# seanome/kmerseek

Hardware: NVIDIA B200
Metric: residues/s sketched+indexed (higher is better)
Workload: dtype u64

## Files before the change

### kmerseek_b200/csrc/dense.cu

```cuda
#include <cub/device/device_radix_sort.cuh>
#include <cub/device/device_scan.cuh>

#include <algorithm>
#include <cmath>

#include "common.cuh"
#include "dense.cuh"
#include "dense_scatter.cuh"
#include "index_build.cuh"
#include "sketch.cuh"

namespace ks {

namespace {

__device__ uint64_t murmur_of_pattern(uint32_t pattern, uint32_t k) {
    uint64_t w[3] = {0, 0, 0};
    for (uint32_t j = 0; j < k; j++) w[j >> 3] |= (uint64_t)(((pattern >> j) & 1u) ? 'h' : 'p') << (8 * (j & 7));
    uint64_t h1 = SEED, h2 = SEED;
    const uint32_t nb = k / 16, rem = k % 16;
    if (nb) {
        h1 ^= mix_k1(w[0]);
        h1 = rotl64(h1, 27) + h2;
        h1 = h1 * 5 + 0x52dce729;
        h2 ^= mix_k2(w[1]);
        h2 = rotl64(h2, 31) + h1;
        h2 = h2 * 5 + 0x38495ab5;
    }
    const uint64_t t1 = w[2 * nb], t2 = nb ? 0 : w[1];
    if (rem > 8) h2 ^= mix_k2(t2);
    if (rem > 0) h1 ^= mix_k1(t1);
    h1 ^= k;
    h2 ^= k;
    h1 += h2;
    h2 += h1;
    h1 = fmix64(h1);
    h2 = fmix64(h2);
    return h1 + h2;
}

__device__ __forceinline__ uint32_t hp_translate(uint32_t c) {
    constexpr uint32_t H = (1u << 0) | (1u << 5) | (1u << 6) | (1u << 8) | (1u << 11) | (1u << 12) | (1u << 15) | (1u << 21) |
                           (1u << 22) | (1u << 24);
    constexpr uint32_t P = (1u << 2) | (1u << 3) | (1u << 4) | (1u << 7) | (1u << 10) | (1u << 13) | (1u << 16) | (1u << 17) |
                           (1u << 18) | (1u << 19);
    if (c == '*') return '*';
    const uint32_t i = c - 'A';
    if (i < 26u) {
        if ((H >> i) & 1u) return 'h';
        if ((P >> i) & 1u) return 'p';
    }
    return 'X';
}

__device__ __noinline__ uint64_t dense_window_hash(const uint8_t* __restrict__ res, int packed, uint64_t g, uint32_t k) {
    uint64_t w[3] = {0, 0, 0};
    for (uint32_t j = 0; j < k; j++) {
        const uint64_t i = g + j;
        uint32_t c;
        if (packed) {
            const uint64_t byte = (i >> 3) * 5;
            uint64_t v = 0;
            for (int t = 0; t < 5; t++) v |= (uint64_t)res[byte + t] << (8 * t);
            const uint32_t code = (uint32_t)(v >> (5 * (i & 7))) & 31u;
            c = code == 0 ? 0u : code <= 26 ? 'A' + code - 1 : code == 27 ? (uint32_t)'*' : 0u;
        } else {
            c = res[i];
        }
        w[j >> 3] |= (uint64_t)hp_translate(c) << (8 * (j & 7));
    }
    uint64_t h1 = SEED, h2 = SEED;
    const uint32_t nb = k / 16, rem = k % 16;
    if (nb) {
        h1 ^= mix_k1(w[0]);
        h1 = rotl64(h1, 27) + h2;
        h1 = h1 * 5 + 0x52dce729;
        h2 ^= mix_k2(w[1]);
        h2 = rotl64(h2, 31) + h1;
        h2 = h2 * 5 + 0x38495ab5;
    }
    const uint64_t t1 = w[2 * nb], t2 = nb ? 0 : w[1];
    if (rem > 8) h2 ^= mix_k2(t2);
    if (rem > 0) h1 ^= mix_k1(t1);
    h1 ^= k;
    h2 ^= k;
    h1 += h2;
    h2 += h1;
    h1 = fmix64(h1);
    h2 = fmix64(h2);
    return h1 + h2;
}

__global__ void dense_hash_codes_kernel(uint32_t k, uint64_t* __restrict__ hash, uint32_t* __restrict__ code) {
    const uint32_t c = blockIdx.x * blockDim.x + threadIdx.x;
    if (c >= (1u << k)) return;
    hash[c] = murmur_of_pattern(c, k);
    code[c] = c;
}

__global__ void dense_group_base_kernel(uint32_t n, const uint64_t* __restrict__ sorted_hash, uint32_t* __restrict__ group_base) {
    const uint32_t p = blockIdx.x * blockDim.x + threadIdx.x;
    if (p > (1u << DENSE_PREFIX_BITS)) return;
    if (p == (1u << DENSE_PREFIX_BITS)) { group_base[p] = n; return; }
    const uint64_t lim = (uint64_t)p << (64 - DENSE_PREFIX_BITS);
    uint32_t lo = 0, hi = n;
    while (lo < hi) {
        const uint32_t mid = (lo + hi) >> 1;
        if (sorted_hash[mid] < lim) lo = mid + 1; else hi = mid;
    }
    group_base[p] = lo;
}

__global__ void dense_check_kernel(uint32_t n, const uint64_t* __restrict__ sorted_hash, const uint32_t* __restrict__ group_base,
                                   uint32_t* __restrict__ flags) {
    const uint32_t r = blockIdx.x * blockDim.x + threadIdx.x;
    if (r >= n) return;
    const uint64_t h = sorted_hash[r];
    if (h == 0 || (r && sorted_hash[r - 1] == h)) atomicOr(flags, 1u);
    atomicMax(flags + 3, r - group_base[(uint32_t)(h >> (64 - DENSE_PREFIX_BITS))]);
}

__global__ void dense_code_kernel(uint32_t n, const uint64_t* __restrict__ sorted_hash, const uint32_t* __restrict__ pattern_of_rank,
                                  const uint32_t* __restrict__ group_base, int rb, int parity, uint32_t* __restrict__ code_of_pattern) {
    const uint32_t r = blockIdx.x * blockDim.x + threadIdx.x;
    if (r >= n) return;
    const uint32_t pfx = (uint32_t)(sorted_hash[r] >> (64 - DENSE_PREFIX_BITS));
    const uint32_t local = r - group_base[pfx];
    code_of_pattern[pattern_of_rank[r]] = (pfx << rb) | (parity ? 2u * local + 1u : local);
}

__global__ void dense_windows_kernel(const uint64_t* __restrict__ offsets, uint32_t n_prot, uint32_t k,
                                     uint32_t* __restrict__ t_abund, uint32_t* __restrict__ t_size) {
    const uint32_t p = blockIdx.x * blockDim.x + threadIdx.x;
    if (p >= n_prot) return;
    const uint64_t len = offsets[p + 1] - offsets[p];
    const uint32_t w = len >= k ? (uint32_t)(len - k + 1) : 0u;
    t_abund[p] = w;
    t_size[p] = w;
}

__device__ __forceinline__ uint64_t hash_of_code(uint32_t code, int rb, int parity, const uint32_t* __restrict__ group_base,
                                                 const uint64_t* __restrict__ sorted_hash) {
    return sorted_hash[group_base[code >> rb] + ((code & ((1u << rb) - 1u)) >> parity)];
}

constexpr int DC_THREADS = 256;
constexpr int DC_ROWS = 8;
constexpr int DC_TILE = DC_THREADS * DC_ROWS;

__global__ void __launch_bounds__(DC_THREADS)
dense_count_kernel(const uint64_t* __restrict__ keys, uint64_t n, int loc_bits, int pos_bits, uint64_t* __restrict__ tile_counts) {
    __shared__ uint32_t s_k[DC_THREADS / 32], s_g[DC_THREADS / 32];
    const uint32_t tid = threadIdx.x, lane = tid & 31, warp = tid >> 5;
    const uint64_t base = (uint64_t)blockIdx.x * DC_TILE;
    uint32_t ck = 0, cg = 0;
#pragma unroll
    for (int r = 0; r < DC_ROWS; r++) {
        const uint64_t i = base + (uint64_t)(warp * DC_ROWS + r) * 32 + lane;
        bool hk = false, hg = false;
        const uint64_t key = i < n ? keys[i] : 0ull;
        uint64_t prev = __shfl_up_sync(0xffffffffu, key, 1);
        if (i < n) {
            if (lane == 0) prev = i ? keys[i - 1] : ~key;
            hk = (key >> loc_bits) != (prev >> loc_bits);
            hg = (key >> pos_bits) != (prev >> pos_bits);
        }
        ck += __popc(__ballot_sync(0xffffffffu, hk));
        cg += __popc(__ballot_sync(0xffffffffu, hg));
    }
    if (lane == 0) { s_k[warp] = ck; s_g[warp] = cg; }
    __syncthreads();
    if (tid == 0) {
        uint32_t k = 0, g = 0;
        for (int w = 0; w < DC_THREADS / 32; w++) { k += s_k[w]; g += s_g[w]; }
        tile_counts[blockIdx.x] = (uint64_t)k | ((uint64_t)g << 32);
        if (blockIdx.x == gridDim.x - 1) tile_counts[gridDim.x] = 0;
    }
}

__global__ void __launch_bounds__(DC_THREADS)
dense_write_kernel(const uint64_t* __restrict__ keys_in, uint64_t n, int loc_bits, int pos_bits, const uint64_t* __restrict__ tile_prefix,
                   const uint64_t* __restrict__ sorted_hash, const uint32_t* __restrict__ group_base, int rb, int parity,
                   uint64_t* __restrict__ loc, uint64_t* __restrict__ keys,
                   uint32_t* __restrict__ key_grp, uint32_t* __restrict__ grp_start, uint32_t* __restrict__ t_size,
                   uint64_t* __restrict__ d_counts) {
    __shared__ uint32_t s_k[DC_THREADS / 32], s_g[DC_THREADS / 32];
    const uint32_t tid = threadIdx.x, lane = tid & 31, warp = tid >> 5;
    const uint32_t lt = (1u << lane) - 1u;
    const uint64_t base = (uint64_t)blockIdx.x * DC_TILE;
    const uint64_t pos_mask = (1ull << pos_bits) - 1ull, pid_mask = (1ull << (loc_bits - pos_bits)) - 1ull;
    uint64_t key[DC_ROWS];
    uint32_t bk[DC_ROWS], bg[DC_ROWS];
    uint32_t wk = 0, wg = 0;
#pragma unroll
    for (int r = 0; r < DC_ROWS; r++) {
        const uint64_t i = base + (uint64_t)(warp * DC_ROWS + r) * 32 + lane;
        bool hk = false, hg = false;
        key[r] = i < n ? keys_in[i] : 0ull;
        uint64_t prev = __shfl_up_sync(0xffffffffu, key[r], 1);
        if (i < n) {
            if (lane == 0) prev = i ? keys_in[i - 1] : ~key[r];
            hk = (key[r] >> loc_bits) != (prev >> loc_bits);
            hg = (key[r] >> pos_bits) != (prev >> pos_bits);
            const uint32_t pid = (uint32_t)((key[r] >> pos_bits) & pid_mask);
            loc[i] = ((uint64_t)pid << 32) | (key[r] & pos_mask);
            if (!hg) atomicSub(&t_size[pid], 1u);
        }
        bk[r] = __ballot_sync(0xffffffffu, hk);
        bg[r] = __ballot_sync(0xffffffffu, hg);
        wk += __popc(bk[r]);
        wg += __popc(bg[r]);
    }
    if (lane == 0) { s_k[warp] = wk; s_g[warp] = wg; }
    __syncthreads();
    const uint64_t pfx = tile_prefix[blockIdx.x];
    uint32_t rk = (uint32_t)pfx, rg = (uint32_t)(pfx >> 32);
    uint32_t tk = 0, tg = 0;
#pragma unroll
    for (int w = 0; w < DC_THREADS / 32; w++) {
        if (w < (int)warp) { rk += s_k[w]; rg += s_g[w]; }
        tk += s_k[w];
        tg += s_g[w];
    }
#pragma unroll
    for (int r = 0; r < DC_ROWS; r++) {
        const uint64_t i = base + (uint64_t)(warp * DC_ROWS + r) * 32 + lane;
        const uint32_t g = rg + __popc(bg[r] & lt);
        if ((bg[r] >> lane) & 1u) grp_start[g] = (uint32_t)i;
        if ((bk[r] >> lane) & 1u) {
            const uint32_t u = rk + __popc(bk[r] & lt);
            keys[u] = hash_of_code((uint32_t)(key[r] >> loc_bits), rb, parity, group_base, sorted_hash);
            key_grp[u] = g;
        }
        rk += __popc(bk[r]);
        rg += __popc(bg[r]);
    }
    if (blockIdx.x == gridDim.x - 1 && tid == 0) {
        const uint64_t U = (uint32_t)pfx + tk, G = (uint32_t)(pfx >> 32) + tg;
        d_counts[0] = U;
        d_counts[1] = G;
        key_grp[U] = (uint32_t)G;
        grp_start[G] = (uint32_t)n;
    }
}

#ifndef KS_DP_CTAS
#define KS_DP_CTAS 5
#endif
__global__ void __launch_bounds__(DS_THREADS, KS_DP_CTAS)
dense_partition_kernel(const uint64_t* __restrict__ region1, uint32_t cap1, const uint2* __restrict__ chunk_map, DenseScatter sc) {
    __shared__ DenseScatterSmem s_sc;
    __shared__ uint64_t s_dst[DS_TILE];
    const uint2 e = chunk_map[blockIdx.x];
    const uint32_t nv = e.x >> 16, b1 = e.x & 0xffffu;
    if (nv == 0) return;
    const uint64_t* src = region1 + (uint64_t)b1 * cap1 + e.y;
    uint64_t key[DS_ITEMS];
    uint32_t valid = 0;
#pragma unroll
    for (int it = 0; it < DS_ITEMS; it++) {
        const uint32_t i = it * DS_THREADS + threadIdx.x;
        key[it] = 0;
        if (i < nv) { key[it] = src[i]; valid |= 1u << it; }
    }
    scatter_keys(key, valid, sc, b1 << sc.bits, s_sc, s_dst);
}

#ifndef KS_DB_THREADS
#define KS_DB_THREADS 512
#endif
constexpr int DB_THREADS = KS_DB_THREADS;
constexpr int DB_CTAS = 2048 / DB_THREADS;
constexpr int DB_WARPS = DB_THREADS / 32;
constexpr int DB_CAP = 4096;
constexpr int DB_ROWS = DB_CAP / DB_THREADS;
constexpr int DB_BIN_BITS = 13;
constexpr int DB_BINS = 1 << DB_BIN_BITS;
constexpr int DB_WORDS_PER_THREAD = DB_BINS / 2 / DB_THREADS;
#ifdef KS_DB_NOSLICE
constexpr int DB_HASH_SLICE = 0;
#else
constexpr int DB_HASH_SLICE = 512;
#endif
constexpr size_t DB_SMEM = (size_t)DB_CAP * 8 + (size_t)DB_BINS * 2 + (size_t)DB_HASH_SLICE * 8;
constexpr uint32_t DB_BIN_SORT_MAX = 32;
constexpr int DB_SLOT_BITS = 12;
static_assert(DB_WORDS_PER_THREAD % 4 == 0 && DB_ROWS * DB_WARPS == 128, "scan layout");

struct DenseBucketArgs {
    const uint64_t* region2;
    const uint32_t* cursor2;
    const uint32_t* bstart;
    uint32_t nb;
    int bucket_bits;
    int rem_bits;
    int loc_bits, pos_bits;
    int rb, parity;
    const uint64_t* sorted_hash;
    const uint32_t* group_base;
    uint64_t* loc;
    uint64_t* keys;
    uint32_t *key_grp, *grp_start, *t_size;
    uint64_t* counts;
    unsigned long long* d_counts;
    uint32_t* dir;
    int dir_sub, dir_shift;
    const uint8_t* residues;
    const uint64_t* offsets;
    int packed;
    uint32_t k;
    const uint32_t* exc_flag;
    const uint32_t* skip_flag;
};

template <bool EXC>
__global__ void __launch_bounds__(DB_THREADS, DB_CTAS)
dense_bucket_kernel(DenseBucketArgs a) {
    extern __shared__ __align__(16) unsigned char smem_raw[];
    uint64_t* B = reinterpret_cast<uint64_t*>(smem_raw);
    uint32_t* cnt = reinterpret_cast<uint32_t*>(B + DB_CAP);
    uint64_t* s_hash = reinterpret_cast<uint64_t*>(cnt + DB_BINS / 2);
    uint64_t* s_keyh = reinterpret_cast<uint64_t*>(cnt);
    constexpr uint32_t KEYH_CAP = DB_BINS / 4;
    const uint16_t* off16 = reinterpret_cast<const uint16_t*>(cnt);
    __shared__ uint32_t s_wsum[DB_WARPS];
    __shared__ uint32_t s_cw[DB_ROWS * DB_WARPS];
    __shared__ uint32_t s_tk, s_tg;
    const uint32_t tid = threadIdx.x, lane = tid & 31, warp = tid >> 5;
    const uint32_t lt = (1u << lane) - 1u;
    if (*a.skip_flag != 0) return;
    if ((*a.exc_flag != 0) != EXC) return;
    const int up = 64 - a.rem_bits;
    const int rrb = a.rem_bits - a.loc_bits;
    const int pb = up + a.loc_bits;
    const bool squeeze = a.parity && pb >= 64 - DB_BIN_BITS && pb < 63;
    const int n_low = squeeze ? DB_BIN_BITS - (63 - pb) : 0;
    auto bin_of = [&](uint64_t it) -> uint32_t {
        if (!squeeze) return (uint32_t)(it >> (64 - DB_BIN_BITS));
        return (uint32_t)(((it >> (pb + 1)) << n_low) | ((it >> (pb - n_low)) & ((1ull << n_low) - 1ull)));
    };
    const int rank_sh = up + a.loc_bits, grp_sh = up + a.pos_bits;
    const uint64_t pos_mask = (1ull << a.pos_bits) - 1ull, pid_mask = (1ull << (a.loc_bits - a.pos_bits)) - 1ull;
    constexpr uint64_t SLOT_MASK = (1ull << DB_SLOT_BITS) - 1ull;
    const uint32_t dir_n = 1u << a.dir_sub;
    auto dir_local = [&](uint64_t h) -> int32_t { return (int32_t)((uint32_t)(h >> a.dir_shift) & (dir_n - 1u)); };
    for (uint32_t b = blockIdx.x; b < a.nb; b += gridDim.x) {
    __syncthreads();
    for (uint32_t i = tid; i < DB_BINS / 8; i += DB_THREADS) reinterpret_cast<uint4*>(cnt)[i] = make_uint4(0, 0, 0, 0);
    const uint64_t* src = a.region2 + (uint64_t)b * DB_CAP;
    uint64_t item[DB_ROWS];
    constexpr int SPEC_ROWS = DB_ROWS / 2;
#pragma unroll
    for (int r = 0; r < SPEC_ROWS; r++) item[r] = src[r * DB_THREADS + tid];
    const uint32_t m = min(a.cursor2[b], (uint32_t)DB_CAP);
    const uint32_t s0 = a.bstart[b];
    const uint32_t kb = s0 + b;
    uint32_t* dir_b = a.dir + (uint64_t)b * (dir_n + 1u);
    const uint32_t pshift = DENSE_PREFIX_BITS - a.bucket_bits;
    const uint32_t slice_base = a.group_base[b << pshift];
    const uint32_t slice_n = a.group_base[(b + 1) << pshift] - slice_base;
    const bool hash_slice = DB_HASH_SLICE > 0 && slice_n <= (uint32_t)DB_HASH_SLICE;
    if (hash_slice) for (uint32_t i = tid; i < slice_n; i += DB_THREADS) s_hash[i] = a.sorted_hash[slice_base + i];
    if (m == 0) {
        if (tid == 0) { a.key_grp[kb] = kb; a.grp_start[kb] = s0; a.counts[b] = 0; }
        for (uint32_t x = tid; x <= dir_n; x += DB_THREADS) dir_b[x] = kb;
        continue;
    }
#pragma unroll
    for (int r = SPEC_ROWS; r < DB_ROWS; r++) {
        if (r * DB_THREADS >= m) break;
        const uint32_t j = r * DB_THREADS + tid;
        if (j < m) item[r] = src[j];
    }
    __syncthreads();
#pragma unroll
    for (int r = 0; r < DB_ROWS; r++) {
        const uint32_t j = r * DB_THREADS + tid;
        if (r * DB_THREADS >= m) break;
        if (j < m) {
            item[r] <<= up;
            const uint32_t bin = bin_of(item[r]), sh16 = 16 * (bin & 1u);
            item[r] |= (atomicAdd(&cnt[bin >> 1], 1u << sh16) >> sh16) & 0xffffu;
        }
    }
    __syncthreads();
    bool big_bin = false;
    {
        uint32_t w[DB_WORDS_PER_THREAD];
#pragma unroll
        for (int q = 0; q < DB_WORDS_PER_THREAD / 4; q++) {
            const uint4 c = reinterpret_cast<uint4*>(cnt)[tid * (DB_WORDS_PER_THREAD / 4) + q];
            w[4 * q] = c.x; w[4 * q + 1] = c.y; w[4 * q + 2] = c.z; w[4 * q + 3] = c.w;
        }
        uint32_t total = 0;
#pragma unroll
        for (int i = 0; i < DB_WORDS_PER_THREAD; i++) {
            const uint32_t lo = w[i] & 0xffffu, hi = w[i] >> 16;
            total += lo + hi;
            big_bin |= lo > DB_BIN_SORT_MAX || hi > DB_BIN_SORT_MAX;
        }
        uint32_t incl = total;
#pragma unroll
        for (int o = 1; o < 32; o <<= 1) {
            const uint32_t v = __shfl_up_sync(0xffffffffu, incl, o);
            if ((int)lane >= o) incl += v;
        }
        if (lane == 31) s_wsum[warp] = incl;
        __syncthreads();
        uint32_t off = 0;
#pragma unroll
        for (int w2 = 0; w2 < DB_WARPS; w2++) off += w2 < (int)warp ? s_wsum[w2] : 0u;
        uint32_t run = off + incl - total;
#pragma unroll
        for (int i = 0; i < DB_WORDS_PER_THREAD; i++) {
            const uint32_t lo = w[i] & 0xffffu, hi = w[i] >> 16;
            w[i] = run | ((run + lo) << 16);
            run += lo + hi;
        }
#pragma unroll
        for (int q = 0; q < DB_WORDS_PER_THREAD / 4; q++)
            reinterpret_cast<uint4*>(cnt)[tid * (DB_WORDS_PER_THREAD / 4) + q] = make_uint4(w[4 * q], w[4 * q + 1], w[4 * q + 2], w[4 * q + 3]);
    }
    __syncthreads();
#pragma unroll
    for (int r = 0; r < DB_ROWS; r++) {
        const uint32_t j = r * DB_THREADS + tid;
        if (r * DB_THREADS >= m) break;
        if (j < m) B[off16[bin_of(item[r])] + (uint32_t)(item[r] & SLOT_MASK)] = item[r];
    }
#ifdef KS_DB_RANKSORT
    const int use_rounds = __syncthreads_or((EXC || big_bin) ? 1 : 0);
#else
    (void)big_bin;
    const int use_rounds = __syncthreads_or(1);
#endif
    if (!use_rounds) {
#pragma unroll
        for (int r = 0; r < DB_ROWS; r++) {
            const uint32_t j = r * DB_THREADS + tid;
            if (r * DB_THREADS >= m) break;
            if (j < m) {
                const uint32_t bin = bin_of(item[r]);
                const uint32_t lo = off16[bin], hi = bin == DB_BINS - 1 ? m : off16[bin + 1];
                uint32_t at = lo;
                for (uint32_t t = lo; t < hi; t++) at += B[t] < item[r] ? 1u : 0u;
                item[r] = (item[r] & ~SLOT_MASK) | at;
            }
        }
        __syncthreads();
#pragma unroll
        for (int r = 0; r < DB_ROWS; r++) {
            const uint32_t j = r * DB_THREADS + tid;
            if (r * DB_THREADS >= m) break;
            if (j < m) B[(uint32_t)(item[r] & SLOT_MASK)] = item[r];
        }
        __syncthreads();
    } else {
        const uint32_t np0 = m >> 1, np1 = (m - 1) >> 1;
        ulonglong2* B2 = reinterpret_cast<ulonglong2*>(B);
        int again;
        do {
            int sw = 0;
            for (uint32_t i = tid; i < np0; i += DB_THREADS) {
                const ulonglong2 v = B2[i];
                if (v.x > v.y) { B2[i] = make_ulonglong2(v.y, v.x); sw = 1; }
            }
            __syncthreads();
            for (uint32_t i = tid; i < np1; i += DB_THREADS) {
                const uint64_t x = B[2 * i + 1], y = B[2 * i + 2];
                if (x > y) { B[2 * i + 1] = y; B[2 * i + 2] = x; sw = 1; }
            }
            again = __syncthreads_or(sw);
        } while (again);
    }
    auto is_exc = [&](uint64_t it) -> bool { return ((it >> rank_sh) & 1ull) == 0ull; };
    auto hash_of = [&](uint64_t it) -> uint64_t {
        const uint64_t low = it >> up;
        const uint32_t pid = (uint32_t)((low >> a.pos_bits) & pid_mask);
        return dense_window_hash(a.residues, a.packed, a.offsets[pid] + (low & pos_mask), a.k);
    };
    if (EXC) {
        for (uint32_t j = tid; j < m; j += DB_THREADS) {
            const uint64_t it = B[j];
            if (!is_exc(it) || (j && (B[j - 1] >> rank_sh) == (it >> rank_sh))) continue;
            uint32_t e = j + 1;
            while (e < m && (B[e] >> rank_sh) == (it >> rank_sh)) e++;
            if (e - j < 2) continue;
            const uint64_t h0 = hash_of(it);
            bool mixed = false;
            for (uint32_t t = j + 1; t < e && !mixed; t++) mixed = hash_of(B[t]) != h0;
            if (!mixed) continue;
            for (uint32_t t = j + 1; t < e; t++) {
                const uint64_t x = B[t], hx = hash_of(x);
                uint32_t u = t;
                while (u > j) {
                    const uint64_t y = B[u - 1], hy = hash_of(y);
                    if (hy < hx || (hy == hx && y < x)) break;
                    B[u] = y;
                    u--;
                }
                B[u] = x;
            }
        }
        __syncthreads();
    }
    uint32_t flags = 0;
#pragma unroll
    for (int r = 0; r < DB_ROWS; r++) {
        const uint32_t j = r * DB_THREADS + tid;
        if (r * DB_THREADS < m) {
            bool hk = false, hg = false;
            if (j < m) {
                const uint64_t it = B[j];
                const uint64_t pv = j ? B[j - 1] : ~it;
                hk = j == 0 || (it >> rank_sh) != (pv >> rank_sh);
                if (EXC && !hk && is_exc(it)) hk = hash_of(it) != hash_of(pv);
                hg = hk || (it >> grp_sh) != (pv >> grp_sh);
                const uint64_t low = it >> up;
                const uint32_t pid = (uint32_t)((low >> a.pos_bits) & pid_mask);
                a.loc[s0 + j] = ((uint64_t)pid << 32) | (low & pos_mask);
                if (!hg) atomicSub(&a.t_size[pid], 1u);
            }
            flags |= ((hk ? 1u : 0u) | (hg ? 2u : 0u)) << (2 * r);
            const uint32_t ck = __popc(__ballot_sync(0xffffffffu, hk)), cg = __popc(__ballot_sync(0xffffffffu, hg));
            if (lane == 0) s_cw[r * DB_WARPS + warp] = ck | (cg << 16);
        } else if (lane == 0) {
            s_cw[r * DB_WARPS + warp] = 0;
        }
    }
    __syncthreads();
    if (warp == 0) {
        uint32_t v[4], local = 0;
#pragma unroll
        for (int i = 0; i < 4; i++) { v[i] = s_cw[lane * 4 + i]; local += v[i]; }
        uint32_t incl = local;
#pragma unroll
        for (int o = 1; o < 32; o <<= 1) {
            const uint32_t t = __shfl_up_sync(0xffffffffu, incl, o);
            if ((int)lane >= o) incl += t;
        }
        uint32_t run = incl - local;
#pragma unroll
        for (int i = 0; i < 4; i++) { s_cw[lane * 4 + i] = run; run += v[i]; }
        const uint32_t tot = __shfl_sync(0xffffffffu, incl, 31);
        if (lane == 0) {
            const uint32_t tk = tot & 0xffffu, tg = tot >> 16;
            s_tk = tk; s_tg = tg;
            a.counts[b] = (uint64_t)tk | ((uint64_t)tg << 32);
            atomicAdd(a.d_counts, (unsigned long long)tk);
            atomicAdd(a.d_counts + 1, (unsigned long long)tg);
        }
    }
    __syncthreads();
    const uint32_t tk = s_tk, tg = s_tg;
    const uint32_t code_top = b << rrb;
#pragma unroll
    for (int r = 0; r < DB_ROWS; r++) {
        if (r * DB_THREADS < m) {
            const uint32_t j = r * DB_THREADS + tid;
            const bool hk = (flags >> (2 * r)) & 1u, hg = (flags >> (2 * r)) & 2u;
            const uint32_t bk = __ballot_sync(0xffffffffu, hk), bg = __ballot_sync(0xffffffffu, hg);
            const uint32_t pre = s_cw[r * DB_WARPS + warp];
            const uint32_t g = kb + (pre >> 16) + __popc(bg & lt);
            if (hg) a.grp_start[g] = s0 + j;
            if (hk) {
                const uint32_t ul = (pre & 0xffffu) + __popc(bk & lt);
                const uint64_t it = B[j];
                uint64_t h;
                if (EXC && is_exc(it)) {
                    h = hash_of(it);
                } else {
                    const uint32_t code = code_top | (uint32_t)(it >> rank_sh);
                    const uint32_t gb = pshift == 0 ? slice_base : a.group_base[code >> a.rb];
                    const uint32_t idx = gb + ((code & ((1u << a.rb) - 1u)) >> a.parity);
                    h = hash_slice ? s_hash[idx - slice_base] : a.sorted_hash[idx];
                }
                a.keys[kb + ul] = h;
                a.key_grp[kb + ul] = g;
                if (tk <= KEYH_CAP) s_keyh[ul] = h;
            }
            if (j == m - 1) {
                a.key_grp[kb + tk] = kb + tg;
                a.grp_start[kb + tg] = s0 + m;
            }
        }
    }
    __syncthreads();
    for (uint32_t i = tid; i < tk; i += DB_THREADS) {
        const uint64_t h = tk <= KEYH_CAP ? s_keyh[i] : a.keys[kb + i];
        const int32_t x1 = dir_local(h);
        int32_t x0 = -1;
        if (i) x0 = dir_local(tk <= KEYH_CAP ? s_keyh[i - 1] : a.keys[kb + i - 1]);
        for (int32_t x = x0 + 1; x <= x1; x++) dir_b[x] = kb + i;
        if (i == tk - 1) for (int32_t x = x1 + 1; x <= (int32_t)dir_n; x++) dir_b[x] = kb + tk;
    }
    }
}

size_t align256(size_t b) { return (b + 255) & ~(size_t)255; }

size_t table_sort_bytes(uint32_t n) {
    size_t b = 0;
    cub::DeviceRadixSort::SortPairs(nullptr, b, (const uint64_t*)nullptr, (uint64_t*)nullptr, (const uint32_t*)nullptr,
                                    (uint32_t*)nullptr, (int64_t)n, 0, 64);
    return align256(b);
}

size_t key_sort_bytes(uint64_t n) {
    size_t b = 0;
    cub::DoubleBuffer<uint64_t> k(nullptr, nullptr);
    cub::DeviceRadixSort::SortKeys(nullptr, b, k, (int64_t)n, 0, 64);
    return align256(b);
}

size_t scan_bytes(uint64_t n) {
    size_t b = 0;
    cub::DeviceScan::ExclusiveSum(nullptr, b, (const uint64_t*)nullptr, (uint64_t*)nullptr, (int64_t)n);
    return align256(b);
}

}

size_t dense_table_temp_bytes(uint32_t k) {
    const size_t n = (size_t)1 << k;
    return align256(n * 8) + 2 * align256(n * 4) + table_sort_bytes((uint32_t)n) + 256;
}

#define KS_TRY(x) do { cudaError_t e_ = (x); if (e_ != cudaSuccess) return e_; } while (0)

cudaError_t dense_build_tables(uint32_t k, uint64_t* sorted_hash, uint32_t* group_base, uint32_t* pattern_of_rank, void* temp,
                               size_t temp_bytes, uint32_t* d_flags, cudaStream_t stream, uint64_t* n_launches) {
    const uint32_t n = 1u << k;
    if (temp_bytes < dense_table_temp_bytes(k)) return cudaErrorInvalidValue;
    char* p = (char*)temp;
    uint64_t* hash = (uint64_t*)p; p += align256((size_t)n * 8);
    uint32_t* code = (uint32_t*)p; p += align256((size_t)n * 4);
    size_t sort_bytes = table_sort_bytes(n);
    KS_TRY(cudaMemsetAsync(d_flags, 0, 4, stream));
    KS_TRY(cudaMemsetAsync(d_flags + 3, 0, 4, stream));
    dense_hash_codes_kernel<<<(n + 255) / 256, 256, 0, stream>>>(k, hash, code);
    KS_TRY(cudaGetLastError());
    KS_TRY(cub::DeviceRadixSort::SortPairs(p, sort_bytes, hash, sorted_hash, code, pattern_of_rank, (int64_t)n, 0, 64, stream));
    dense_group_base_kernel<<<((1u << DENSE_PREFIX_BITS) + 1 + 255) / 256, 256, 0, stream>>>(n, sorted_hash, group_base);
    dense_check_kernel<<<(n + 255) / 256, 256, 0, stream>>>(n, sorted_hash, group_base, d_flags);
    if (n_launches) *n_launches += 3 + 10;
    return cudaGetLastError();
}

cudaError_t dense_build_codes(uint32_t k, const uint64_t* sorted_hash, const uint32_t* group_base, const uint32_t* pattern_of_rank,
                              int rb, int parity, uint32_t* code_of_pattern, cudaStream_t stream, uint64_t* n_launches) {
    const uint32_t n = 1u << k;
    dense_code_kernel<<<(n + 255) / 256, 256, 0, stream>>>(n, sorted_hash, pattern_of_rank, group_base, rb, parity, code_of_pattern);
    if (n_launches) *n_launches += 1;
    return cudaGetLastError();
}

DenseSortPlan dense_sort_plan(uint64_t n, int rank_bits, int key_bits, int k) {
    DenseSortPlan p;
    int total = 0;
    while (total <= 2 * DS_MAX_BITS && (n >> total) > 3072) total++;
    if ((double)n / std::ldexp(1.0, k) > 1024.0) return p;
    while (total < DENSE_PREFIX_BITS) {
        const double lambda = std::ldexp(1.0, k - total), per_pattern = (double)n / std::ldexp(1.0, k);
        if (lambda * per_pattern + 6.0 * per_pattern * std::sqrt(lambda > 1.0 ? lambda : 1.0) <= (double)DB_CAP) break;
        total++;
    }
    if (total > 2 * DS_MAX_BITS || total > DENSE_PREFIX_BITS || total > rank_bits || n == 0) return p;
    if (key_bits - total > 64 - DB_SLOT_BITS) return p;
    p.custom = 1;
    p.total = total;
    p.l1 = total < DS_MAX_BITS ? total : DS_MAX_BITS;
    p.l2 = total - p.l1;
    p.cap1 = p.l2 ? (uint32_t)((n >> p.l1) + (n >> (p.l1 + 3)) + 16384) : (uint32_t)DB_CAP;
    size_t off = 0;
    auto take = [&](size_t bytes) { const size_t o = off; off += align256(bytes); return o; };
    p.off_region1 = take(((size_t)p.cap1 << p.l1) * 8);
    p.off_region2 = p.l2 ? take(((size_t)DB_CAP << total) * 8) : p.off_region1;
    p.off_small = off;
    p.off_cursor1 = take(((size_t)1 << p.l1) * 4);
    p.off_cursor2 = p.l2 ? take(((size_t)1 << total) * 4) : p.off_cursor1;
    p.off_overflow = take(8);
    p.small_bytes = off - p.off_small;
    p.max_chunks = (uint32_t)(n / DS_TILE + ((size_t)1 << p.l1) + 1);
    p.off_chunks = take((size_t)p.max_chunks * 8);
    p.off_bstart = take((((size_t)1 << total) + 1) * 4);
    p.off_counts = take(((size_t)1 << total) * 8);
    p.bytes = off;
    return p;
}

size_t dense_csr_temp_bytes(uint64_t n) {
    const uint64_t nt = (n + DC_TILE - 1) / DC_TILE;
    return key_sort_bytes(n) + 2 * align256((nt + 1) * 8) + scan_bytes(nt + 1) + 256;
}

cudaError_t dense_build_csr(const DenseCsrArgs& a, cudaStream_t stream, uint64_t* sort_launches, uint64_t* csr_launches) {
    if (a.out_dir_sub) *a.out_dir_sub = DIR_SUB_COMPACT;
    if (a.out_seg_nb) *a.out_seg_nb = 0;
    const uint64_t n = a.n;
    const int loc_bits = a.pid_bits + a.pos_bits;
    if (a.n_prot) {
        dense_windows_kernel<<<(a.n_prot + 255) / 256, 256, 0, stream>>>(a.offsets, a.n_prot, a.k, a.t_abund, a.t_size);
        KS_TRY(cudaGetLastError());
        if (csr_launches) *csr_launches += 1;
    }
    if (n == 0) {
        KS_TRY(cudaMemsetAsync(a.d_counts, 0, 16, stream));
        KS_TRY(cudaMemsetAsync(a.key_grp, 0, 4, stream));
        KS_TRY(cudaMemsetAsync(a.grp_start, 0, 4, stream));
        if (a.ev_sorted) KS_TRY(cudaEventRecord(a.ev_sorted, stream));
        return cudaSuccess;
    }
    if (a.plan.custom) {
        const DenseSortPlan& pl = a.plan;
        char* w = (char*)a.work;
        uint64_t* region1 = (uint64_t*)(w + pl.off_region1);
        uint64_t* region2 = (uint64_t*)(w + pl.off_region2);
        uint32_t* cursor1 = (uint32_t*)(w + pl.off_cursor1);
        uint32_t* cursor2 = (uint32_t*)(w + pl.off_cursor2);
        uint2* chunk_map = (uint2*)(w + pl.off_chunks);
        uint32_t* bstart = (uint32_t*)(w + pl.off_bstart);
        const uint32_t nb = 1u << pl.total;
        const int total_bits = a.rank_bits + loc_bits;
        if (pl.l2) {
            dense_chunks_kernel<<<1, 256, 0, stream>>>(cursor1, 1u << pl.l1, pl.cap1, chunk_map, pl.max_chunks);
            DenseScatter sc;
            sc.out = region2; sc.cursor = cursor2; sc.cap = (uint32_t)DB_CAP; sc.shift = total_bits - pl.total; sc.bits = pl.l2;
            sc.overflow = a.overflow ? a.overflow : (uint32_t*)(w + pl.off_overflow);
            dense_partition_kernel<<<pl.max_chunks, DS_THREADS, 0, stream>>>(region1, pl.cap1, chunk_map, sc);
            KS_TRY(cudaGetLastError());
            if (sort_launches) *sort_launches += 2;
        }
        dense_bucket_offsets_kernel<<<1, 1024, 0, stream>>>(cursor2, nb, (uint32_t)DB_CAP, bstart);
        if (a.ev_sorted) KS_TRY(cudaEventRecord(a.ev_sorted, stream));
        if (a.dir_bits < pl.total) return cudaErrorInvalidValue;
        if (!a.counts_zeroed) KS_TRY(cudaMemsetAsync(a.d_counts, 0, 16, stream));
        DenseBucketArgs ba;
        ba.region2 = region2; ba.cursor2 = cursor2; ba.bstart = bstart; ba.nb = nb; ba.bucket_bits = pl.total;
        ba.rem_bits = total_bits - pl.total; ba.loc_bits = loc_bits; ba.pos_bits = a.pos_bits; ba.rb = a.rb; ba.parity = a.parity;
        ba.sorted_hash = a.sorted_hash; ba.group_base = a.group_base;
        ba.loc = a.loc; ba.keys = a.keys; ba.key_grp = a.key_grp; ba.grp_start = a.grp_start; ba.t_size = a.t_size;
        ba.counts = (uint64_t*)(w + pl.off_counts); ba.d_counts = (unsigned long long*)a.d_counts;
        ba.dir = a.dir; ba.dir_sub = a.dir_bits - pl.total; ba.dir_shift = 64 - a.dir_bits;
        ba.residues = a.residues; ba.offsets = a.offsets; ba.packed = a.packed; ba.k = a.k;
        ba.exc_flag = a.exc_flag; ba.skip_flag = a.skip_flag;
        static thread_local int attr_device = -1;
        int dev = 0;
        KS_TRY(cudaGetDevice(&dev));
        if (attr_device != dev) {
            KS_TRY(cudaFuncSetAttribute(dense_bucket_kernel<true>, cudaFuncAttributeMaxDynamicSharedMemorySize, (int)DB_SMEM));
            KS_TRY(cudaFuncSetAttribute(dense_bucket_kernel<false>, cudaFuncAttributeMaxDynamicSharedMemorySize, (int)DB_SMEM));
            attr_device = dev;
        }
        dense_bucket_kernel<false><<<nb, DB_THREADS, DB_SMEM, stream>>>(ba);
        dense_bucket_kernel<true><<<std::min<unsigned>(nb, 148u * DB_CTAS), DB_THREADS, DB_SMEM, stream>>>(ba);
        if (sort_launches) *sort_launches += 3;
        if (a.out_dir_sub) *a.out_dir_sub = ba.dir_sub;
        if (a.out_seg_nb) *a.out_seg_nb = nb;
        if (a.out_seg_start) *a.out_seg_start = bstart;
        if (a.out_seg_counts) *a.out_seg_counts = ba.counts;
        return cudaGetLastError();
    }
    char* p = (char*)a.temp;
    size_t sort_bytes = key_sort_bytes(n);
    void* sort_temp = p; p += sort_bytes;
    const uint64_t nt = (n + DC_TILE - 1) / DC_TILE;
    uint64_t* tile_counts = (uint64_t*)p; p += align256((nt + 1) * 8);
    uint64_t* tile_prefix = (uint64_t*)p; p += align256((nt + 1) * 8);
    size_t sbytes = scan_bytes(nt + 1);
    void* scan_temp = p;
    cub::DoubleBuffer<uint64_t> kb(a.keys_a, a.keys_b);
    KS_TRY(cub::DeviceRadixSort::SortKeys(sort_temp, sort_bytes, kb, (int64_t)n, loc_bits, loc_bits + a.rank_bits, stream));
    if (sort_launches) *sort_launches += 2 + (a.rank_bits + 7) / 8;
    if (a.ev_sorted) KS_TRY(cudaEventRecord(a.ev_sorted, stream));
    const uint64_t* sorted = kb.Current();
    dense_count_kernel<<<(unsigned)nt, DC_THREADS, 0, stream>>>(sorted, n, loc_bits, a.pos_bits, tile_counts);
    KS_TRY(cudaGetLastError());
    KS_TRY(cub::DeviceScan::ExclusiveSum(scan_temp, sbytes, tile_counts, tile_prefix, (int64_t)(nt + 1), stream));
    dense_write_kernel<<<(unsigned)nt, DC_THREADS, 0, stream>>>(sorted, n, loc_bits, a.pos_bits, tile_prefix, a.sorted_hash, a.group_base,
                                                                a.rb, a.parity, a.loc, a.keys, a.key_grp, a.grp_start, a.t_size, a.d_counts);
    if (csr_launches) *csr_launches += 4;
    if (a.out_dir_sub) *a.out_dir_sub = DIR_SUB_COMPACT;
    if (a.out_seg_nb) *a.out_seg_nb = 0;
    return cudaGetLastError();
#undef KS_TRY
}

}
```

Before: 39.25 billion.

## Sort 32-bit index keys in dense bucket kernel instead of 64-bit items

The per-bucket shared-memory sort now works on 32-bit words that pack the top 20 sort bits with a 12-bit item index, which halves the shared item buffer, and full 64-bit keys are re-read from global memory via __ldg when needed. Runs of equal prefixes are finished with a per-run insertion sort using the real keys. Buckets with oversized bins fall back to a bitonic sort on 64-bit words. It also force-inlines the window hash and uses warp shuffles for neighbour comparisons. This cuts shared-memory footprint and traffic, but adds indirect global loads and extra tie-breaking work.

```diff
diff --git a/kmerseek_b200/csrc/dense.cu b/kmerseek_b200/csrc/dense.cu
--- a/kmerseek_b200/csrc/dense.cu
+++ b/kmerseek_b200/csrc/dense.cu
@@ -53,7 +53,7 @@
     return 'X';
 }
 
-__device__ __noinline__ uint64_t dense_window_hash(const uint8_t* __restrict__ res, int packed, uint64_t g, uint32_t k) {
+__device__ __forceinline__ uint64_t dense_window_hash(const uint8_t* __restrict__ res, int packed, uint64_t g, uint32_t k) {
     uint64_t w[3] = {0, 0, 0};
     for (uint32_t j = 0; j < k; j++) {
         const uint64_t i = g + j;
@@ -282,10 +282,12 @@
 #else
 constexpr int DB_HASH_SLICE = 512;
 #endif
-constexpr size_t DB_SMEM = (size_t)DB_CAP * 8 + (size_t)DB_BINS * 2 + (size_t)DB_HASH_SLICE * 8;
+constexpr int DB_IDX_BITS = 12;
+constexpr uint32_t DB_IDX_MASK = (1u << DB_IDX_BITS) - 1u;
+constexpr size_t DB_SMEM = (size_t)DB_CAP * 4 + (size_t)DB_BINS * 2 + (size_t)DB_HASH_SLICE * 8;
 constexpr uint32_t DB_BIN_SORT_MAX = 32;
-constexpr int DB_SLOT_BITS = 12;
 static_assert(DB_WORDS_PER_THREAD % 4 == 0 && DB_ROWS * DB_WARPS == 128, "scan layout");
+static_assert(DB_CAP == 1 << DB_IDX_BITS && DB_BINS * 2 == DB_CAP * 4, "items and counters are one 64-bit array of DB_CAP");
 
 struct DenseBucketArgs {
     const uint64_t* region2;
@@ -317,9 +319,10 @@
 __global__ void __launch_bounds__(DB_THREADS, DB_CTAS)
 dense_bucket_kernel(DenseBucketArgs a) {
     extern __shared__ __align__(16) unsigned char smem_raw[];
-    uint64_t* B = reinterpret_cast<uint64_t*>(smem_raw);
-    uint32_t* cnt = reinterpret_cast<uint32_t*>(B + DB_CAP);
+    uint32_t* I = reinterpret_cast<uint32_t*>(smem_raw);
+    uint32_t* cnt = I + DB_CAP;
     uint64_t* s_hash = reinterpret_cast<uint64_t*>(cnt + DB_BINS / 2);
+    uint64_t* W = reinterpret_cast<uint64_t*>(smem_raw);
     uint64_t* s_keyh = reinterpret_cast<uint64_t*>(cnt);
     constexpr uint32_t KEYH_CAP = DB_BINS / 4;
     const uint16_t* off16 = reinterpret_cast<const uint16_t*>(cnt);
@@ -331,27 +334,27 @@
     if (*a.skip_flag != 0) return;
     if ((*a.exc_flag != 0) != EXC) return;
     const int up = 64 - a.rem_bits;
-    const int rrb = a.rem_bits - a.loc_bits;
-    const int pb = up + a.loc_bits;
-    const bool squeeze = a.parity && pb >= 64 - DB_BIN_BITS && pb < 63;
-    const int n_low = squeeze ? DB_BIN_BITS - (63 - pb) : 0;
-    auto bin_of = [&](uint64_t it) -> uint32_t {
-        if (!squeeze) return (uint32_t)(it >> (64 - DB_BIN_BITS));
-        return (uint32_t)(((it >> (pb + 1)) << n_low) | ((it >> (pb - n_low)) & ((1ull << n_low) - 1ull)));
+    auto sort_bits = [&](uint64_t key) -> uint32_t { return (uint32_t)((key << up) >> 32) & ~DB_IDX_MASK; };
+    const int pb = up + a.loc_bits - 32;
+    const bool squeeze = a.parity && pb >= 32 - DB_BIN_BITS && pb < 31;
+    const int n_low = squeeze ? DB_BIN_BITS - (31 - pb) : 0;
+    auto bin_of = [&](uint32_t it) -> uint32_t {
+        if (!squeeze) return it >> (32 - DB_BIN_BITS);
+        return ((it >> (pb + 1)) << n_low) | ((it >> (pb - n_low)) & ((1u << n_low) - 1u));
     };
-    const int rank_sh = up + a.loc_bits, grp_sh = up + a.pos_bits;
-    const uint64_t pos_mask = (1ull << a.pos_bits) - 1ull, pid_mask = (1ull << (a.loc_bits - a.pos_bits)) - 1ull;
-    constexpr uint64_t SLOT_MASK = (1ull << DB_SLOT_BITS) - 1ull;
+    auto pid_of = [&](uint64_t key) -> uint32_t { return (uint32_t)((key >> a.pos_bits) & ((1ull << (a.loc_bits - a.pos_bits)) - 1ull)); };
+    auto pos_of = [&](uint64_t key) -> uint64_t { return key & ((1ull << a.pos_bits) - 1ull); };
     const uint32_t dir_n = 1u << a.dir_sub;
     auto dir_local = [&](uint64_t h) -> int32_t { return (int32_t)((uint32_t)(h >> a.dir_shift) & (dir_n - 1u)); };
     for (uint32_t b = blockIdx.x; b < a.nb; b += gridDim.x) {
-    __syncthreads();
+    if (b != blockIdx.x) __syncthreads();
     for (uint32_t i = tid; i < DB_BINS / 8; i += DB_THREADS) reinterpret_cast<uint4*>(cnt)[i] = make_uint4(0, 0, 0, 0);
     const uint64_t* src = a.region2 + (uint64_t)b * DB_CAP;
-    uint64_t item[DB_ROWS];
+    auto key_at = [&](uint32_t j) -> uint64_t { return __ldg(src + (I[j] & DB_IDX_MASK)); };
+    uint32_t item[DB_ROWS];
     constexpr int SPEC_ROWS = DB_ROWS / 2;
 #pragma unroll
-    for (int r = 0; r < SPEC_ROWS; r++) item[r] = src[r * DB_THREADS + tid];
+    for (int r = 0; r < SPEC_ROWS; r++) item[r] = sort_bits(src[r * DB_THREADS + tid]);
     const uint32_t m = min(a.cursor2[b], (uint32_t)DB_CAP);
     const uint32_t s0 = a.bstart[b];
     const uint32_t kb = s0 + b;
@@ -370,7 +373,7 @@
     for (int r = SPEC_ROWS; r < DB_ROWS; r++) {
         if (r * DB_THREADS >= m) break;
         const uint32_t j = r * DB_THREADS + tid;
-        if (j < m) item[r] = src[j];
+        if (j < m) item[r] = sort_bits(src[j]);
     }
     __syncthreads();
 #pragma unroll
@@ -378,7 +381,6 @@
         const uint32_t j = r * DB_THREADS + tid;
         if (r * DB_THREADS >= m) break;
         if (j < m) {
-            item[r] <<= up;
             const uint32_t bin = bin_of(item[r]), sh16 = 16 * (bin & 1u);
             item[r] |= (atomicAdd(&cnt[bin >> 1], 1u << sh16) >> sh16) & 0xffffu;
         }
@@ -386,18 +388,18 @@
     __syncthreads();
     bool big_bin = false;
     {
-        uint32_t w[DB_WORDS_PER_THREAD];
+        uint4* c4 = reinterpret_cast<uint4*>(cnt) + tid * (DB_WORDS_PER_THREAD / 4);
+        uint32_t total = 0;
 #pragma unroll
         for (int q = 0; q < DB_WORDS_PER_THREAD / 4; q++) {
-            const uint4 c = reinterpret_cast<uint4*>(cnt)[tid * (DB_WORDS_PER_THREAD / 4) + q];
-            w[4 * q] = c.x; w[4 * q + 1] = c.y; w[4 * q + 2] = c.z; w[4 * q + 3] = c.w;
-        }
-        uint32_t total = 0;
-#pragma unroll
-        for (int i = 0; i < DB_WORDS_PER_THREAD; i++) {
-            const uint32_t lo = w[i] & 0xffffu, hi = w[i] >> 16;
-            total += lo + hi;
-            big_bin |= lo > DB_BIN_SORT_MAX || hi > DB_BIN_SORT_MAX;
+            const uint4 c = c4[q];
+            const uint32_t w[4] = {c.x, c.y, c.z, c.w};
+#pragma unroll
+            for (int i = 0; i < 4; i++) {
+                const uint32_t lo = w[i] & 0xffffu, hi = w[i] >> 16;
+                total += lo + hi;
+                big_bin |= lo > DB_BIN_SORT_MAX || hi > DB_BIN_SORT_MAX;
+            }
         }
         uint32_t incl = total;
 #pragma unroll
@@ -412,94 +414,128 @@
         for (int w2 = 0; w2 < DB_WARPS; w2++) off += w2 < (int)warp ? s_wsum[w2] : 0u;
         uint32_t run = off + incl - total;
 #pragma unroll
-        for (int i = 0; i < DB_WORDS_PER_THREAD; i++) {
-            const uint32_t lo = w[i] & 0xffffu, hi = w[i] >> 16;
-            w[i] = run | ((run + lo) << 16);
-            run += lo + hi;
-        }
-#pragma unroll
-        for (int q = 0; q < DB_WORDS_PER_THREAD / 4; q++)
-            reinterpret_cast<uint4*>(cnt)[tid * (DB_WORDS_PER_THREAD / 4) + q] = make_uint4(w[4 * q], w[4 * q + 1], w[4 * q + 2], w[4 * q + 3]);
-    }
-    __syncthreads();
-#pragma unroll
-    for (int r = 0; r < DB_ROWS; r++) {
-        const uint32_t j = r * DB_THREADS + tid;
-        if (r * DB_THREADS >= m) break;
-        if (j < m) B[off16[bin_of(item[r])] + (uint32_t)(item[r] & SLOT_MASK)] = item[r];
-    }
-#ifdef KS_DB_RANKSORT
-    const int use_rounds = __syncthreads_or((EXC || big_bin) ? 1 : 0);
-#else
-    (void)big_bin;
-    const int use_rounds = __syncthreads_or(1);
-#endif
-    if (!use_rounds) {
+        for (int q = 0; q < DB_WORDS_PER_THREAD / 4; q++) {
+            const uint4 c = c4[q];
+            uint32_t w[4] = {c.x, c.y, c.z, c.w};
+#pragma unroll
+            for (int i = 0; i < 4; i++) {
+                const uint32_t lo = w[i] & 0xffffu, hi = w[i] >> 16;
+                w[i] = run | ((run + lo) << 16);
+                run += lo + hi;
+            }
+            c4[q] = make_uint4(w[0], w[1], w[2], w[3]);
+        }
+    }
+    if (!__syncthreads_or(big_bin ? 1 : 0)) {
 #pragma unroll
         for (int r = 0; r < DB_ROWS; r++) {
             const uint32_t j = r * DB_THREADS + tid;
             if (r * DB_THREADS >= m) break;
-            if (j < m) {
-                const uint32_t bin = bin_of(item[r]);
-                const uint32_t lo = off16[bin], hi = bin == DB_BINS - 1 ? m : off16[bin + 1];
-                uint32_t at = lo;
-                for (uint32_t t = lo; t < hi; t++) at += B[t] < item[r] ? 1u : 0u;
-                item[r] = (item[r] & ~SLOT_MASK) | at;
-            }
+            if (j < m) I[off16[bin_of(item[r])] + (item[r] & DB_IDX_MASK)] = (item[r] & ~DB_IDX_MASK) | j;
         }
         __syncthreads();
-#pragma unroll
-        for (int r = 0; r < DB_ROWS; r++) {
-            const uint32_t j = r * DB_THREADS + tid;
-            if (r * DB_THREADS >= m) break;
-            if (j < m) B[(uint32_t)(item[r] & SLOT_MASK)] = item[r];
-        }
-        __syncthreads();
-    } else {
         const uint32_t np0 = m >> 1, np1 = (m - 1) >> 1;
-        ulonglong2* B2 = reinterpret_cast<ulonglong2*>(B);
+        uint2* I2 = reinterpret_cast<uint2*>(I);
         int again;
         do {
             int sw = 0;
             for (uint32_t i = tid; i < np0; i += DB_THREADS) {
-                const ulonglong2 v = B2[i];
-                if (v.x > v.y) { B2[i] = make_ulonglong2(v.y, v.x); sw = 1; }
+                const uint2 v = I2[i];
+                if (v.x > v.y) { I2[i] = make_uint2(v.y, v.x); sw = 1; }
             }
             __syncthreads();
             for (uint32_t i = tid; i < np1; i += DB_THREADS) {
-                const uint64_t x = B[2 * i + 1], y = B[2 * i + 2];
-                if (x > y) { B[2 * i + 1] = y; B[2 * i + 2] = x; sw = 1; }
+                const uint32_t x = I[2 * i + 1], y = I[2 * i + 2];
+                if (x > y) { I[2 * i + 1] = y; I[2 * i + 2] = x; sw = 1; }
             }
             again = __syncthreads_or(sw);
         } while (again);
-    }
-    auto is_exc = [&](uint64_t it) -> bool { return ((it >> rank_sh) & 1ull) == 0ull; };
-    auto hash_of = [&](uint64_t it) -> uint64_t {
-        const uint64_t low = it >> up;
-        const uint32_t pid = (uint32_t)((low >> a.pos_bits) & pid_mask);
-        return dense_window_hash(a.residues, a.packed, a.offsets[pid] + (low & pos_mask), a.k);
+        for (uint32_t j = tid + 1; j < m; j += DB_THREADS) {
+            const uint32_t it = I[j], pv = I[j - 1];
+            if ((it ^ pv) >> DB_IDX_BITS) continue;
+            if (j >= 2 && ((I[j - 2] ^ pv) >> DB_IDX_BITS) == 0) continue;
+            uint32_t e = j + 1;
+            while (e < m && ((I[e] ^ it) >> DB_IDX_BITS) == 0) e++;
+            for (uint32_t t = j; t < e; t++) {
+                const uint32_t x = I[t];
+                const uint64_t kx = __ldg(src + (x & DB_IDX_MASK));
+                uint32_t u = t;
+                while (u > j - 1) {
+                    const uint32_t y = I[u - 1];
+                    if (__ldg(src + (y & DB_IDX_MASK)) < kx) break;
+                    I[u] = y;
+                    u--;
+                }
+                I[u] = x;
+            }
+        }
+        __syncthreads();
+    } else {
+#pragma unroll
+        for (int r = 0; r < DB_ROWS; r++) {
+            const uint32_t j = r * DB_THREADS + tid;
+            if (j < m) W[j] = (src[j] << up) | j;
+        }
+        __syncthreads();
+        uint32_t n2 = 2;
+        while (n2 < m) n2 <<= 1;
+        for (uint32_t size = 2; size <= n2; size <<= 1) {
+            for (uint32_t stride = size >> 1; stride > 0; stride >>= 1) {
+                for (uint32_t t = tid; t < n2 / 2; t += DB_THREADS) {
+                    const uint32_t lo = 2 * t - (t & (stride - 1u));
+                    const uint32_t hi = stride == size >> 1 ? lo ^ (size - 1u) : lo + stride;
+                    if (hi < m) {
+                        const uint64_t x = W[lo], y = W[hi];
+                        if (x > y) { W[lo] = y; W[hi] = x; }
+                    }
+                }
+                __syncthreads();
+            }
+        }
+#pragma unroll
+        for (int r = 0; r < DB_ROWS; r++) {
+            const uint32_t j = r * DB_THREADS + tid;
+            if (j < m) {
+                const uint64_t w = W[j];
+                item[r] = ((uint32_t)(w >> 32) & ~DB_IDX_MASK) | ((uint32_t)w & DB_IDX_MASK);
+            }
+        }
+        __syncthreads();
+#pragma unroll
+        for (int r = 0; r < DB_ROWS; r++) {
+            const uint32_t j = r * DB_THREADS + tid;
+            if (j < m) I[j] = item[r];
+        }
+        __syncthreads();
+    }
+    auto is_exc = [&](uint64_t key) -> bool { return ((key >> a.loc_bits) & 1ull) == 0ull; };
+    auto hash_of = [&](uint64_t key) -> uint64_t {
+        return dense_window_hash(a.residues, a.packed, a.offsets[pid_of(key)] + pos_of(key), a.k);
     };
     if (EXC) {
         for (uint32_t j = tid; j < m; j += DB_THREADS) {
-            const uint64_t it = B[j];
-            if (!is_exc(it) || (j && (B[j - 1] >> rank_sh) == (it >> rank_sh))) continue;
+            const uint64_t key = key_at(j);
+            const uint64_t code = key >> a.loc_bits;
+            if (!is_exc(key) || (j && (key_at(j - 1) >> a.loc_bits) == code)) continue;
             uint32_t e = j + 1;
-            while (e < m && (B[e] >> rank_sh) == (it >> rank_sh)) e++;
+            while (e < m && (key_at(e) >> a.loc_bits) == code) e++;
             if (e - j < 2) continue;
-            const uint64_t h0 = hash_of(it);
+            const uint64_t h0 = hash_of(key);
             bool mixed = false;
-            for (uint32_t t = j + 1; t < e && !mixed; t++) mixed = hash_of(B[t]) != h0;
+            for (uint32_t t = j + 1; t < e && !mixed; t++) mixed = hash_of(key_at(t)) != h0;
             if (!mixed) continue;
             for (uint32_t t = j + 1; t < e; t++) {
-                const uint64_t x = B[t], hx = hash_of(x);
+                const uint32_t xi = I[t];
+                const uint64_t x = __ldg(src + (xi & DB_IDX_MASK)), hx = hash_of(x);
                 uint32_t u = t;
                 while (u > j) {
-                    const uint64_t y = B[u - 1], hy = hash_of(y);
+                    const uint32_t yi = I[u - 1];
+                    const uint64_t y = __ldg(src + (yi & DB_IDX_MASK)), hy = hash_of(y);
                     if (hy < hx || (hy == hx && y < x)) break;
-                    B[u] = y;
+                    I[u] = yi;
                     u--;
                 }
-                B[u] = x;
+                I[u] = xi;
             }
         }
         __syncthreads();
@@ -510,15 +546,15 @@
         const uint32_t j = r * DB_THREADS + tid;
         if (r * DB_THREADS < m) {
             bool hk = false, hg = false;
+            const uint64_t key = j < m ? key_at(j) : 0ull;
+            uint64_t pv = __shfl_up_sync(0xffffffffu, key, 1);
             if (j < m) {
-                const uint64_t it = B[j];
-                const uint64_t pv = j ? B[j - 1] : ~it;
-                hk = j == 0 || (it >> rank_sh) != (pv >> rank_sh);
-                if (EXC && !hk && is_exc(it)) hk = hash_of(it) != hash_of(pv);
-                hg = hk || (it >> grp_sh) != (pv >> grp_sh);
-                const uint64_t low = it >> up;
-                const uint32_t pid = (uint32_t)((low >> a.pos_bits) & pid_mask);
-                a.loc[s0 + j] = ((uint64_t)pid << 32) | (low & pos_mask);
+                if (lane == 0) pv = j ? key_at(j - 1) : ~key;
+                hk = j == 0 || (key >> a.loc_bits) != (pv >> a.loc_bits);
+                if (EXC && !hk && is_exc(key)) hk = hash_of(key) != hash_of(pv);
+                hg = hk || (key >> a.pos_bits) != (pv >> a.pos_bits);
+                const uint32_t pid = pid_of(key);
+                a.loc[s0 + j] = ((uint64_t)pid << 32) | pos_of(key);
                 if (!hg) atomicSub(&a.t_size[pid], 1u);
             }
             flags |= ((hk ? 1u : 0u) | (hg ? 2u : 0u)) << (2 * r);
@@ -553,7 +589,6 @@
     }
     __syncthreads();
     const uint32_t tk = s_tk, tg = s_tg;
-    const uint32_t code_top = b << rrb;
 #pragma unroll
     for (int r = 0; r < DB_ROWS; r++) {
         if (r * DB_THREADS < m) {
@@ -565,12 +600,12 @@
             if (hg) a.grp_start[g] = s0 + j;
             if (hk) {
                 const uint32_t ul = (pre & 0xffffu) + __popc(bk & lt);
-                const uint64_t it = B[j];
+                const uint64_t key = key_at(j);
                 uint64_t h;
-                if (EXC && is_exc(it)) {
-                    h = hash_of(it);
+                if (EXC && is_exc(key)) {
+                    h = hash_of(key);
                 } else {
-                    const uint32_t code = code_top | (uint32_t)(it >> rank_sh);
+                    const uint32_t code = (uint32_t)(key >> a.loc_bits);
                     const uint32_t gb = pshift == 0 ? slice_base : a.group_base[code >> a.rb];
                     const uint32_t idx = gb + ((code & ((1u << a.rb) - 1u)) >> a.parity);
                     h = hash_slice ? s_hash[idx - slice_base] : a.sorted_hash[idx];
@@ -666,7 +701,7 @@
         total++;
     }
     if (total > 2 * DS_MAX_BITS || total > DENSE_PREFIX_BITS || total > rank_bits || n == 0) return p;
-    if (key_bits - total > 64 - DB_SLOT_BITS) return p;
+    if (key_bits - total > 64 - DB_IDX_BITS) return p;
     p.custom = 1;
     p.total = total;
     p.l1 = total < DS_MAX_BITS ? total : DS_MAX_BITS;
```

Measured after the change: 39.32 billion (median of 6 runs). No clear change (+0.2%).
